# cure-lab/MagicDrive

Measured on NVIDIA H100. Metric: 6-view 224x400 denoising-steps/sec, higher is better.
Workload: dtype bf16

## Files before the change

### magicdrive_b200/csrc/attention_wgmma.cuh

```cuda
#pragma once
#include "ptx.cuh"
#include "wgmma.cuh"

namespace mdb {

constexpr int ATT_BM = 128;

constexpr int ATT_MAX_SRC = 3;
struct AttnKvMaps {
  CUtensorMap k[ATT_MAX_SRC], v[ATT_MAX_SRC];
};

struct AttnParams {
  __nv_bfloat16* out;
  int ldo;
  int lq, lk;
  const int* kv_index;
  int n_sets;
  const int* kv_len;
  int n_src;
  float scale_log2;
  int q_step;
};

template <int D, int BN_ = 0>
struct AttnCfg {
  static constexpr int KD = (D + 63) / 64;
  static constexpr int D16 = (D + 15) / 16 * 16;
  static constexpr int BN = BN_ ? BN_ : ((D16 <= 64) ? 128 : 64);
  static constexpr int TILE_Q = ATT_BM * 128;
  static constexpr int TILE_KV = BN * 128;
  static constexpr int SMEM_Q = KD * TILE_Q;
  static constexpr int STAGES_FIT = (232448 - 1024 - 256 - SMEM_Q) / (2 * KD * TILE_KV);
  static constexpr int STAGES = STAGES_FIT > 4 ? 4 : STAGES_FIT;
  static constexpr int SMEM_KV = STAGES * 2 * KD * TILE_KV;
  static constexpr int kSmemBytes = SMEM_Q + SMEM_KV + 1024 + 256;
  static constexpr int kConsumerWarps = 8;
  static constexpr int kThreads = 32 * kConsumerWarps + 32;
  static constexpr int SACC = BN / 2;
  static constexpr int OACC = D16 / 2;
  static_assert(STAGES >= 1 && kSmemBytes <= 232448, "shared memory");
};

template <int D, int BN_, bool CAUSAL = false>
__global__ void __launch_bounds__(AttnCfg<D, BN_>::kThreads, 1)
attention_wgmma_kernel(const __grid_constant__ CUtensorMap tmQ, const __grid_constant__ AttnKvMaps kvm, const AttnParams p) {
  using Cfg = AttnCfg<D, BN_>;
  constexpr int KD = Cfg::KD, D16 = Cfg::D16, BN = Cfg::BN, STAGES = Cfg::STAGES;
  constexpr int TILE_Q = Cfg::TILE_Q, TILE_KV = Cfg::TILE_KV;
  extern __shared__ uint8_t smem_raw[];
  uint8_t* smem = reinterpret_cast<uint8_t*>((reinterpret_cast<uintptr_t>(smem_raw) + 1023) & ~uintptr_t(1023));
  uint8_t* smQ = smem;
  uint8_t* smK = smQ + Cfg::SMEM_Q;
  uint8_t* smV = smK + STAGES * KD * TILE_KV;
  uint64_t* bars = reinterpret_cast<uint64_t*>(smV + STAGES * KD * TILE_KV);
  uint64_t* q_full = bars;
  uint64_t* q_empty = bars + 1;
  uint64_t* kv_full = bars + 2;
  uint64_t* kv_empty = bars + 2 + STAGES;

  const int warp = threadIdx.x >> 5, lane = threadIdx.x & 31;
  const int b = blockIdx.z, head = blockIdx.y;
  const int nq = (p.lq + ATT_BM - 1) / ATT_BM;
  const int q_step = p.q_step > 0 ? p.q_step : nq;
  const int n_own = (nq - static_cast<int>(blockIdx.x) + q_step - 1) / q_step;
  auto q0_of = [&](int o) { return (static_cast<int>(blockIdx.x) + o * q_step) * ATT_BM; };

  if (warp == Cfg::kConsumerWarps && lane == 0) {
    prefetch_tmap(&tmQ);
    for (int i = 0; i < p.n_src; ++i) {
      prefetch_tmap(&kvm.k[i]);
      prefetch_tmap(&kvm.v[i]);
    }
    mbar_init(q_full, 1);
    mbar_init(q_empty, Cfg::kConsumerWarps);
    for (int i = 0; i < STAGES; ++i) {
      mbar_init(&kv_full[i], 1);
      mbar_init(&kv_empty[i], Cfg::kConsumerWarps);
    }
    fence_barrier_init();
  }
  __syncthreads();
  asm volatile("griddepcontrol.wait;" ::: "memory");
  asm volatile("griddepcontrol.launch_dependents;" ::: "memory");
  const int lkb = p.kv_len ? min(max(p.kv_len[b], 0), p.lk) : p.lk;
  const int ntiles = (lkb + BN - 1) / BN;
  const bool kv_resident = ntiles == 1 && p.n_sets == 1 && n_own > 1;
  auto kv_entry = [&](int set) { return p.kv_index ? p.kv_index[b * p.n_sets + set] : b; };
  auto tiles_of = [&](int kve, int q0) {
    return kve < 0 ? 0 : CAUSAL ? min(ntiles, (min(q0 + ATT_BM, p.lq) - 1) / BN + 1) : ntiles;
  };

  if (warp == Cfg::kConsumerWarps) {
    if (lane == 0) {
      int stage = 0;
      uint32_t phase = 0;
      for (int o = 0; o < n_own; ++o) {
        if (o > 0) mbar_wait(q_empty, static_cast<uint32_t>(o - 1) & 1u);
        mbar_arrive_expect_tx(q_full, KD * TILE_Q);
#pragma unroll
        for (int c = 0; c < KD; ++c) tma_load_4d(&tmQ, q_full, smQ + c * TILE_Q, c * 64, head, q0_of(o), b);
        if (kv_resident && o > 0) continue;
        for (int set = 0; set < p.n_sets; ++set) {
          const int kve = kv_entry(set);
          const int nt = tiles_of(kve, q0_of(o));
          if (nt == 0) continue;
          const int kvb = kve & 0xffffff;
          const CUtensorMap* km = &kvm.k[kve >> 24];
          const CUtensorMap* vm = &kvm.v[kve >> 24];
          for (int j = 0; j < nt; ++j) {
            mbar_wait(&kv_empty[stage], phase ^ 1);
            mbar_arrive_expect_tx(&kv_full[stage], 2 * KD * TILE_KV);
#pragma unroll
            for (int c = 0; c < KD; ++c) {
              tma_load_4d(km, &kv_full[stage], smK + (stage * KD + c) * TILE_KV, c * 64, head, j * BN, kvb);
              tma_load_4d(vm, &kv_full[stage], smV + (stage * KD + c) * TILE_KV, c * 64, head, j * BN, kvb);
            }
            if (++stage == STAGES) {
              stage = 0;
              phase ^= 1;
            }
          }
        }
      }
    }
    return;
  }

  const int wg = warp >> 2;
  const int q = lane & 3;
  const int rloc = 64 * wg + 16 * (warp & 3) + (lane >> 2);
  const float sc = p.scale_log2;
  int stage = 0;
  uint32_t phase = 0;
  for (int o = 0; o < n_own; ++o) {
    const int q0 = q0_of(o);
    mbar_wait(q_full, static_cast<uint32_t>(o) & 1u);
    bool wrote = false;
    for (int set = 0; set < p.n_sets; ++set) {
      const int nt = tiles_of(kv_entry(set), q0);
      if (nt == 0) continue;
      float oacc[Cfg::OACC];
#pragma unroll
      for (int i = 0; i < Cfg::OACC; ++i) oacc[i] = 0.f;
      float m[2] = {-INFINITY, -INFINITY}, l[2] = {0.f, 0.f};
      for (int j = 0; j < nt; ++j) {
        const int st = kv_resident ? 0 : stage;
        mbar_wait(&kv_full[st], kv_resident ? 0u : phase);
        float s[Cfg::SACC];
        wgmma_fence();
#pragma unroll
        for (int k = 0; k < D16 / 16; ++k) {
          const int c = k / 4, kk = k % 4;
          const uint64_t adesc = make_sw128_kmajor_desc(smem_u32(smQ + c * TILE_Q + wg * (64 * 128))) + 2 * kk;
          const uint64_t bdesc = make_sw128_kmajor_desc(smem_u32(smK + (st * KD + c) * TILE_KV)) + 2 * kk;
          WgmmaSS<BN>::run(s, adesc, bdesc, k > 0 ? 1u : 0u);
        }
        wgmma_commit();
        wgmma_wait<0>();
        const int kbase = j * BN;
        if (kbase + BN > lkb) {
#pragma unroll
          for (int g = 0; g < BN / 8; ++g)
#pragma unroll
            for (int e = 0; e < 2; ++e)
              if (kbase + 8 * g + 2 * q + e >= lkb) s[4 * g + e] = s[4 * g + 2 + e] = -INFINITY;
        }
        if constexpr (CAUSAL) {
          if (kbase + BN - 1 > q0 + rloc) {
#pragma unroll
            for (int g = 0; g < BN / 8; ++g)
#pragma unroll
              for (int h = 0; h < 2; ++h)
#pragma unroll
                for (int e = 0; e < 2; ++e)
                  if (kbase + 8 * g + 2 * q + e > q0 + rloc + 8 * h) s[4 * g + 2 * h + e] = -INFINITY;
          }
        }
        float corr[2];
#pragma unroll
        for (int h = 0; h < 2; ++h) {
          float mx = -INFINITY;
#pragma unroll
          for (int g = 0; g < BN / 8; ++g) mx = fmaxf(mx, fmaxf(s[4 * g + 2 * h], s[4 * g + 2 * h + 1]));
          mx = fmaxf(mx, __shfl_xor_sync(0xffffffffu, mx, 1));
          mx = fmaxf(mx, __shfl_xor_sync(0xffffffffu, mx, 2));
          const float m_new = fmaxf(m[h], mx * sc);
          corr[h] = exp2f(m[h] - m_new);
          m[h] = m_new;
        }
        uint32_t pa[BN / 16][4];
        float rs[2] = {0.f, 0.f};
#pragma unroll
        for (int kk = 0; kk < BN / 16; ++kk) {
#pragma unroll
          for (int r = 0; r < 4; ++r) {
            const int h = r & 1;
            const int i0 = 8 * kk + 4 * (r >> 1) + 2 * h;
            const float p0 = exp2f(fmaf(s[i0], sc, -m[h]));
            const float p1 = exp2f(fmaf(s[i0 + 1], sc, -m[h]));
            rs[h] += p0 + p1;
            pa[kk][r] = pack_bf16(p0, p1);
          }
        }
#pragma unroll
        for (int h = 0; h < 2; ++h) l[h] = l[h] * corr[h] + rs[h];
#pragma unroll
        for (int g = 0; g < D16 / 8; ++g) {
          oacc[4 * g] *= corr[0], oacc[4 * g + 1] *= corr[0];
          oacc[4 * g + 2] *= corr[1], oacc[4 * g + 3] *= corr[1];
        }
        wgmma_fence();
#pragma unroll
        for (int kk = 0; kk < BN / 16; ++kk) {
          const uint64_t bdesc = make_sw128_mnmajor_desc(smem_u32(smV + st * KD * TILE_KV), TILE_KV) + (2048u >> 4) * kk;
          WgmmaRSBmn<D16>::run(oacc, pa[kk], bdesc, 1u);
        }
        wgmma_commit();
        wgmma_wait<0>();
        if (!kv_resident) {
          if (lane == 0) mbar_arrive(&kv_empty[stage]);
          if (++stage == STAGES) {
            stage = 0;
            phase ^= 1;
          }
        }
      }
#pragma unroll
      for (int h = 0; h < 2; ++h) {
        l[h] += __shfl_xor_sync(0xffffffffu, l[h], 1);
        l[h] += __shfl_xor_sync(0xffffffffu, l[h], 2);
      }
      const float inv[2] = {1.0f / l[0], 1.0f / l[1]};
#pragma unroll
      for (int h = 0; h < 2; ++h) {
        const int qrow = q0 + rloc + 8 * h;
        if (qrow >= p.lq) continue;
        __nv_bfloat16* orow = p.out + (static_cast<long long>(b) * p.lq + qrow) * p.ldo + head * D;
#pragma unroll
        for (int g = 0; g < D16 / 8; ++g) {
          const int col = 8 * g + 2 * q;
          if (col >= D) continue;
          float f0 = oacc[4 * g + 2 * h] * inv[h], f1 = oacc[4 * g + 2 * h + 1] * inv[h];
          if (wrote) {
            const float2 pf = __bfloat1622float2(*reinterpret_cast<const __nv_bfloat162*>(orow + col));
            f0 = __bfloat162float(__float2bfloat16_rn(f0)) + pf.x;
            f1 = __bfloat162float(__float2bfloat16_rn(f1)) + pf.y;
          }
          *reinterpret_cast<uint32_t*>(orow + col) = pack_bf16(f0, f1);
        }
      }
      wrote = true;
    }
    if (!wrote) {
#pragma unroll
      for (int h = 0; h < 2; ++h) {
        const int qrow = q0 + rloc + 8 * h;
        if (qrow >= p.lq) continue;
        __nv_bfloat16* orow = p.out + (static_cast<long long>(b) * p.lq + qrow) * p.ldo + head * D;
#pragma unroll
        for (int g = 0; g < D16 / 8; ++g)
          if (8 * g + 2 * q < D) *reinterpret_cast<uint32_t*>(orow + 8 * g + 2 * q) = 0u;
      }
    }
    __syncwarp();
    if (lane == 0) mbar_arrive(q_empty);
  }
}

}
```

### magicdrive_b200/csrc/ptx.cuh

```cuda
#pragma once
#include <cuda.h>
#include <cuda_bf16.h>
#include <cuda_runtime.h>
#include <stdint.h>

namespace mdb {

__device__ __forceinline__ uint32_t smem_u32(const void* p) {
  return static_cast<uint32_t>(__cvta_generic_to_shared(p));
}

__device__ __forceinline__ bool elect_one() {
  uint32_t pred = 0;
  asm volatile(
      "{\n\t"
      ".reg .pred P;\n\t"
      "elect.sync _|P, 0xffffffff;\n\t"
      "selp.b32 %0, 1, 0, P;\n\t"
      "}\n"
      : "=r"(pred));
  return pred != 0;
}

__device__ __forceinline__ void mbar_init(uint64_t* bar, uint32_t count) {
  asm volatile("mbarrier.init.shared::cta.b64 [%0], %1;" ::"r"(smem_u32(bar)), "r"(count));
}
__device__ __forceinline__ void fence_barrier_init() {
  asm volatile("fence.mbarrier_init.release.cluster;" ::: "memory");
}
__device__ __forceinline__ void fence_proxy_async() {
  asm volatile("fence.proxy.async.shared::cta;" ::: "memory");
}
__device__ __forceinline__ bool mbar_test(uint64_t* bar, uint32_t parity) {
  uint32_t ok;
  asm volatile(
      "{\n\t"
      ".reg .pred P1;\n\t"
      "mbarrier.test_wait.parity.shared::cta.b64 P1, [%1], %2;\n\t"
      "selp.u32 %0, 1, 0, P1;\n\t"
      "}\n"
      : "=r"(ok)
      : "r"(smem_u32(bar)), "r"(parity)
      : "memory");
  return ok != 0;
}
__device__ __forceinline__ void mbar_arrive_expect_tx(uint64_t* bar, uint32_t bytes) {
  asm volatile("mbarrier.arrive.expect_tx.shared::cta.b64 _, [%0], %1;" ::"r"(smem_u32(bar)), "r"(bytes)
               : "memory");
}
__device__ __forceinline__ void mbar_arrive(uint64_t* bar) {
  asm volatile("mbarrier.arrive.shared::cta.b64 _, [%0];" ::"r"(smem_u32(bar)) : "memory");
}
#ifndef MDB_MBAR_WAIT_MODE
#define MDB_MBAR_WAIT_MODE 0
#endif
__device__ __forceinline__ void mbar_wait(uint64_t* bar, uint32_t parity) {
#if MDB_MBAR_WAIT_MODE == 0
  asm volatile(
      "{\n\t"
      ".reg .pred P1;\n\t"
      "WAIT_LOOP:\n\t"
      "mbarrier.try_wait.parity.shared::cta.b64 P1, [%0], %1, 0x989680;\n\t"
      "@P1 bra DONE;\n\t"
      "bra WAIT_LOOP;\n\t"
      "DONE:\n\t"
      "}\n" ::"r"(smem_u32(bar)),
      "r"(parity)
      : "memory");
#elif MDB_MBAR_WAIT_MODE == 1
  asm volatile(
      "{\n\t"
      ".reg .pred P1;\n\t"
      "WAIT_LOOP:\n\t"
      "mbarrier.try_wait.parity.shared::cta.b64 P1, [%0], %1;\n\t"
      "@P1 bra DONE;\n\t"
      "bra WAIT_LOOP;\n\t"
      "DONE:\n\t"
      "}\n" ::"r"(smem_u32(bar)),
      "r"(parity)
      : "memory");
#else
  asm volatile(
      "{\n\t"
      ".reg .pred P1;\n\t"
      "WAIT_LOOP:\n\t"
      "mbarrier.test_wait.parity.shared::cta.b64 P1, [%0], %1;\n\t"
      "@P1 bra DONE;\n\t"
      "bra WAIT_LOOP;\n\t"
      "DONE:\n\t"
      "}\n" ::"r"(smem_u32(bar)),
      "r"(parity)
      : "memory");
#endif
}

__device__ __forceinline__ void prefetch_tmap(const CUtensorMap* m) {
  asm volatile("prefetch.tensormap [%0];" ::"l"(reinterpret_cast<uint64_t>(m)) : "memory");
}
__device__ __forceinline__ void tma_load_2d(const CUtensorMap* m, uint64_t* bar, void* dst, int c0, int c1) {
  asm volatile(
      "cp.async.bulk.tensor.2d.shared::cluster.global.mbarrier::complete_tx::bytes"
      " [%0], [%1, {%3, %4}], [%2];" ::"r"(smem_u32(dst)),
      "l"(reinterpret_cast<uint64_t>(m)), "r"(smem_u32(bar)), "r"(c0), "r"(c1)
      : "memory");
}
__device__ __forceinline__ void tma_load_4d(const CUtensorMap* m, uint64_t* bar, void* dst, int c0, int c1, int c2,
                                            int c3) {
  asm volatile(
      "cp.async.bulk.tensor.4d.shared::cluster.global.mbarrier::complete_tx::bytes"
      " [%0], [%1, {%3, %4, %5, %6}], [%2];" ::"r"(smem_u32(dst)),
      "l"(reinterpret_cast<uint64_t>(m)), "r"(smem_u32(bar)), "r"(c0), "r"(c1), "r"(c2), "r"(c3)
      : "memory");
}
__device__ __forceinline__ void tma_load_im2col_4d(const CUtensorMap* m, uint64_t* bar, void* dst, int c, int w, int h,
                                                   int n, uint16_t off_w, uint16_t off_h) {
  asm volatile(
      "cp.async.bulk.tensor.4d.shared::cluster.global.im2col.mbarrier::complete_tx::bytes"
      " [%0], [%1, {%3, %4, %5, %6}], [%2], {%7, %8};" ::"r"(smem_u32(dst)),
      "l"(reinterpret_cast<uint64_t>(m)), "r"(smem_u32(bar)), "r"(c), "r"(w), "r"(h), "r"(n), "h"(off_w), "h"(off_h)
      : "memory");
}

__device__ __forceinline__ uint64_t make_sw128_kmajor_desc(uint32_t smem_addr_bytes) {
  uint64_t d = 0;
  d |= static_cast<uint64_t>((smem_addr_bytes >> 4) & 0x3FFF);
  d |= static_cast<uint64_t>(1) << 16;
  d |= static_cast<uint64_t>((1024u >> 4) & 0x3FFF) << 32;
  d |= static_cast<uint64_t>(1) << 62;
  return d;
}
__device__ __forceinline__ uint64_t make_sw128_mnmajor_desc(uint32_t smem_addr_bytes, uint32_t lbo_bytes) {
  uint64_t d = 0;
  d |= static_cast<uint64_t>((smem_addr_bytes >> 4) & 0x3FFF);
  d |= static_cast<uint64_t>((lbo_bytes >> 4) & 0x3FFF) << 16;
  d |= static_cast<uint64_t>((1024u >> 4) & 0x3FFF) << 32;
  d |= static_cast<uint64_t>(1) << 62;
  return d;
}

__device__ __forceinline__ uint32_t pack_bf16(float a, float b) {
  __nv_bfloat162 h = __floats2bfloat162_rn(a, b);
  return *reinterpret_cast<uint32_t*>(&h);
}

}
```

### magicdrive_b200/csrc/wgmma.cuh

```cuda
#pragma once
#include <stdint.h>

namespace mdb {

__device__ __forceinline__ void wgmma_fence() { asm volatile("wgmma.fence.sync.aligned;" ::: "memory"); }
__device__ __forceinline__ void wgmma_commit() { asm volatile("wgmma.commit_group.sync.aligned;" ::: "memory"); }
template <int N>
__device__ __forceinline__ void wgmma_wait() {
  asm volatile("wgmma.wait_group.sync.aligned %0;" ::"n"(N) : "memory");
}

__device__ __forceinline__ void wgmma_ss_n64(float (&d)[32], uint64_t adesc, uint64_t bdesc, uint32_t accumulate) {
  asm volatile(
      "{\n\t.reg .pred p;\n\t"
      "setp.ne.b32 p, %34, 0;\n\t"
      "wgmma.mma_async.sync.aligned.m64n64k16.f32.bf16.bf16 "
      "{%0, %1, %2, %3, %4, %5, %6, %7, %8, %9, %10, %11, %12, %13, %14, %15, %16, %17, %18, %19, %20, %21, %22, %23, %24, %25, %26, %27, %28, %29, %30, %31}, "
      "%32, %33, p, 1, 1, 0, 0;\n\t}\n"
      : "+f"(d[0]), "+f"(d[1]), "+f"(d[2]), "+f"(d[3]), "+f"(d[4]), "+f"(d[5]), "+f"(d[6]), "+f"(d[7]), "+f"(d[8]), "+f"(d[9]), "+f"(d[10]), "+f"(d[11]), "+f"(d[12]), "+f"(d[13]), "+f"(d[14]), "+f"(d[15]), "+f"(d[16]), "+f"(d[17]), "+f"(d[18]), "+f"(d[19]), "+f"(d[20]), "+f"(d[21]), "+f"(d[22]), "+f"(d[23]), "+f"(d[24]), "+f"(d[25]), "+f"(d[26]), "+f"(d[27]), "+f"(d[28]), "+f"(d[29]), "+f"(d[30]), "+f"(d[31])
      : "l"(adesc), "l"(bdesc), "r"(accumulate));
}

__device__ __forceinline__ void wgmma_ss_n128(float (&d)[64], uint64_t adesc, uint64_t bdesc, uint32_t accumulate) {
  asm volatile(
      "{\n\t.reg .pred p;\n\t"
      "setp.ne.b32 p, %66, 0;\n\t"
      "wgmma.mma_async.sync.aligned.m64n128k16.f32.bf16.bf16 "
      "{%0, %1, %2, %3, %4, %5, %6, %7, %8, %9, %10, %11, %12, %13, %14, %15, %16, %17, %18, %19, %20, %21, %22, %23, %24, %25, %26, %27, %28, %29, %30, %31, %32, %33, %34, %35, %36, %37, %38, %39, %40, %41, %42, %43, %44, %45, %46, %47, %48, %49, %50, %51, %52, %53, %54, %55, %56, %57, %58, %59, %60, %61, %62, %63}, "
      "%64, %65, p, 1, 1, 0, 0;\n\t}\n"
      : "+f"(d[0]), "+f"(d[1]), "+f"(d[2]), "+f"(d[3]), "+f"(d[4]), "+f"(d[5]), "+f"(d[6]), "+f"(d[7]), "+f"(d[8]), "+f"(d[9]), "+f"(d[10]), "+f"(d[11]), "+f"(d[12]), "+f"(d[13]), "+f"(d[14]), "+f"(d[15]), "+f"(d[16]), "+f"(d[17]), "+f"(d[18]), "+f"(d[19]), "+f"(d[20]), "+f"(d[21]), "+f"(d[22]), "+f"(d[23]), "+f"(d[24]), "+f"(d[25]), "+f"(d[26]), "+f"(d[27]), "+f"(d[28]), "+f"(d[29]), "+f"(d[30]), "+f"(d[31]), "+f"(d[32]), "+f"(d[33]), "+f"(d[34]), "+f"(d[35]), "+f"(d[36]), "+f"(d[37]), "+f"(d[38]), "+f"(d[39]), "+f"(d[40]), "+f"(d[41]), "+f"(d[42]), "+f"(d[43]), "+f"(d[44]), "+f"(d[45]), "+f"(d[46]), "+f"(d[47]), "+f"(d[48]), "+f"(d[49]), "+f"(d[50]), "+f"(d[51]), "+f"(d[52]), "+f"(d[53]), "+f"(d[54]), "+f"(d[55]), "+f"(d[56]), "+f"(d[57]), "+f"(d[58]), "+f"(d[59]), "+f"(d[60]), "+f"(d[61]), "+f"(d[62]), "+f"(d[63])
      : "l"(adesc), "l"(bdesc), "r"(accumulate));
}

__device__ __forceinline__ void wgmma_ss_n160(float (&d)[80], uint64_t adesc, uint64_t bdesc, uint32_t accumulate) {
  asm volatile(
      "{\n\t.reg .pred p;\n\t"
      "setp.ne.b32 p, %82, 0;\n\t"
      "wgmma.mma_async.sync.aligned.m64n160k16.f32.bf16.bf16 "
      "{%0, %1, %2, %3, %4, %5, %6, %7, %8, %9, %10, %11, %12, %13, %14, %15, %16, %17, %18, %19, %20, %21, %22, %23, %24, %25, %26, %27, %28, %29, %30, %31, %32, %33, %34, %35, %36, %37, %38, %39, %40, %41, %42, %43, %44, %45, %46, %47, %48, %49, %50, %51, %52, %53, %54, %55, %56, %57, %58, %59, %60, %61, %62, %63, %64, %65, %66, %67, %68, %69, %70, %71, %72, %73, %74, %75, %76, %77, %78, %79}, "
      "%80, %81, p, 1, 1, 0, 0;\n\t}\n"
      : "+f"(d[0]), "+f"(d[1]), "+f"(d[2]), "+f"(d[3]), "+f"(d[4]), "+f"(d[5]), "+f"(d[6]), "+f"(d[7]), "+f"(d[8]), "+f"(d[9]), "+f"(d[10]), "+f"(d[11]), "+f"(d[12]), "+f"(d[13]), "+f"(d[14]), "+f"(d[15]), "+f"(d[16]), "+f"(d[17]), "+f"(d[18]), "+f"(d[19]), "+f"(d[20]), "+f"(d[21]), "+f"(d[22]), "+f"(d[23]), "+f"(d[24]), "+f"(d[25]), "+f"(d[26]), "+f"(d[27]), "+f"(d[28]), "+f"(d[29]), "+f"(d[30]), "+f"(d[31]), "+f"(d[32]), "+f"(d[33]), "+f"(d[34]), "+f"(d[35]), "+f"(d[36]), "+f"(d[37]), "+f"(d[38]), "+f"(d[39]), "+f"(d[40]), "+f"(d[41]), "+f"(d[42]), "+f"(d[43]), "+f"(d[44]), "+f"(d[45]), "+f"(d[46]), "+f"(d[47]), "+f"(d[48]), "+f"(d[49]), "+f"(d[50]), "+f"(d[51]), "+f"(d[52]), "+f"(d[53]), "+f"(d[54]), "+f"(d[55]), "+f"(d[56]), "+f"(d[57]), "+f"(d[58]), "+f"(d[59]), "+f"(d[60]), "+f"(d[61]), "+f"(d[62]), "+f"(d[63]), "+f"(d[64]), "+f"(d[65]), "+f"(d[66]), "+f"(d[67]), "+f"(d[68]), "+f"(d[69]), "+f"(d[70]), "+f"(d[71]), "+f"(d[72]), "+f"(d[73]), "+f"(d[74]), "+f"(d[75]), "+f"(d[76]), "+f"(d[77]), "+f"(d[78]), "+f"(d[79])
      : "l"(adesc), "l"(bdesc), "r"(accumulate));
}

__device__ __forceinline__ void wgmma_ss_n256(float (&d)[128], uint64_t adesc, uint64_t bdesc, uint32_t accumulate) {
  asm volatile(
      "{\n\t.reg .pred p;\n\t"
      "setp.ne.b32 p, %130, 0;\n\t"
      "wgmma.mma_async.sync.aligned.m64n256k16.f32.bf16.bf16 "
      "{%0, %1, %2, %3, %4, %5, %6, %7, %8, %9, %10, %11, %12, %13, %14, %15, %16, %17, %18, %19, %20, %21, %22, %23, %24, %25, %26, %27, %28, %29, %30, %31, %32, %33, %34, %35, %36, %37, %38, %39, %40, %41, %42, %43, %44, %45, %46, %47, %48, %49, %50, %51, %52, %53, %54, %55, %56, %57, %58, %59, %60, %61, %62, %63, %64, %65, %66, %67, %68, %69, %70, %71, %72, %73, %74, %75, %76, %77, %78, %79, %80, %81, %82, %83, %84, %85, %86, %87, %88, %89, %90, %91, %92, %93, %94, %95, %96, %97, %98, %99, %100, %101, %102, %103, %104, %105, %106, %107, %108, %109, %110, %111, %112, %113, %114, %115, %116, %117, %118, %119, %120, %121, %122, %123, %124, %125, %126, %127}, "
      "%128, %129, p, 1, 1, 0, 0;\n\t}\n"
      : "+f"(d[0]), "+f"(d[1]), "+f"(d[2]), "+f"(d[3]), "+f"(d[4]), "+f"(d[5]), "+f"(d[6]), "+f"(d[7]), "+f"(d[8]), "+f"(d[9]), "+f"(d[10]), "+f"(d[11]), "+f"(d[12]), "+f"(d[13]), "+f"(d[14]), "+f"(d[15]), "+f"(d[16]), "+f"(d[17]), "+f"(d[18]), "+f"(d[19]), "+f"(d[20]), "+f"(d[21]), "+f"(d[22]), "+f"(d[23]), "+f"(d[24]), "+f"(d[25]), "+f"(d[26]), "+f"(d[27]), "+f"(d[28]), "+f"(d[29]), "+f"(d[30]), "+f"(d[31]), "+f"(d[32]), "+f"(d[33]), "+f"(d[34]), "+f"(d[35]), "+f"(d[36]), "+f"(d[37]), "+f"(d[38]), "+f"(d[39]), "+f"(d[40]), "+f"(d[41]), "+f"(d[42]), "+f"(d[43]), "+f"(d[44]), "+f"(d[45]), "+f"(d[46]), "+f"(d[47]), "+f"(d[48]), "+f"(d[49]), "+f"(d[50]), "+f"(d[51]), "+f"(d[52]), "+f"(d[53]), "+f"(d[54]), "+f"(d[55]), "+f"(d[56]), "+f"(d[57]), "+f"(d[58]), "+f"(d[59]), "+f"(d[60]), "+f"(d[61]), "+f"(d[62]), "+f"(d[63]), "+f"(d[64]), "+f"(d[65]), "+f"(d[66]), "+f"(d[67]), "+f"(d[68]), "+f"(d[69]), "+f"(d[70]), "+f"(d[71]), "+f"(d[72]), "+f"(d[73]), "+f"(d[74]), "+f"(d[75]), "+f"(d[76]), "+f"(d[77]), "+f"(d[78]), "+f"(d[79]), "+f"(d[80]), "+f"(d[81]), "+f"(d[82]), "+f"(d[83]), "+f"(d[84]), "+f"(d[85]), "+f"(d[86]), "+f"(d[87]), "+f"(d[88]), "+f"(d[89]), "+f"(d[90]), "+f"(d[91]), "+f"(d[92]), "+f"(d[93]), "+f"(d[94]), "+f"(d[95]), "+f"(d[96]), "+f"(d[97]), "+f"(d[98]), "+f"(d[99]), "+f"(d[100]), "+f"(d[101]), "+f"(d[102]), "+f"(d[103]), "+f"(d[104]), "+f"(d[105]), "+f"(d[106]), "+f"(d[107]), "+f"(d[108]), "+f"(d[109]), "+f"(d[110]), "+f"(d[111]), "+f"(d[112]), "+f"(d[113]), "+f"(d[114]), "+f"(d[115]), "+f"(d[116]), "+f"(d[117]), "+f"(d[118]), "+f"(d[119]), "+f"(d[120]), "+f"(d[121]), "+f"(d[122]), "+f"(d[123]), "+f"(d[124]), "+f"(d[125]), "+f"(d[126]), "+f"(d[127])
      : "l"(adesc), "l"(bdesc), "r"(accumulate));
}

__device__ __forceinline__ void wgmma_rs_n32_bmn(float (&d)[16], const uint32_t (&a)[4], uint64_t bdesc, uint32_t accumulate) {
  asm volatile(
      "{\n\t.reg .pred p;\n\t"
      "setp.ne.b32 p, %21, 0;\n\t"
      "wgmma.mma_async.sync.aligned.m64n32k16.f32.bf16.bf16 "
      "{%0, %1, %2, %3, %4, %5, %6, %7, %8, %9, %10, %11, %12, %13, %14, %15}, "
      "{%16, %17, %18, %19}, %20, p, 1, 1, 1;\n\t}\n"
      : "+f"(d[0]), "+f"(d[1]), "+f"(d[2]), "+f"(d[3]), "+f"(d[4]), "+f"(d[5]), "+f"(d[6]), "+f"(d[7]), "+f"(d[8]), "+f"(d[9]), "+f"(d[10]), "+f"(d[11]), "+f"(d[12]), "+f"(d[13]), "+f"(d[14]), "+f"(d[15])
      : "r"(a[0]), "r"(a[1]), "r"(a[2]), "r"(a[3]), "l"(bdesc), "r"(accumulate));
}

__device__ __forceinline__ void wgmma_rs_n48_bmn(float (&d)[24], const uint32_t (&a)[4], uint64_t bdesc, uint32_t accumulate) {
  asm volatile(
      "{\n\t.reg .pred p;\n\t"
      "setp.ne.b32 p, %29, 0;\n\t"
      "wgmma.mma_async.sync.aligned.m64n48k16.f32.bf16.bf16 "
      "{%0, %1, %2, %3, %4, %5, %6, %7, %8, %9, %10, %11, %12, %13, %14, %15, %16, %17, %18, %19, %20, %21, %22, %23}, "
      "{%24, %25, %26, %27}, %28, p, 1, 1, 1;\n\t}\n"
      : "+f"(d[0]), "+f"(d[1]), "+f"(d[2]), "+f"(d[3]), "+f"(d[4]), "+f"(d[5]), "+f"(d[6]), "+f"(d[7]), "+f"(d[8]), "+f"(d[9]), "+f"(d[10]), "+f"(d[11]), "+f"(d[12]), "+f"(d[13]), "+f"(d[14]), "+f"(d[15]), "+f"(d[16]), "+f"(d[17]), "+f"(d[18]), "+f"(d[19]), "+f"(d[20]), "+f"(d[21]), "+f"(d[22]), "+f"(d[23])
      : "r"(a[0]), "r"(a[1]), "r"(a[2]), "r"(a[3]), "l"(bdesc), "r"(accumulate));
}

__device__ __forceinline__ void wgmma_rs_n64_bmn(float (&d)[32], const uint32_t (&a)[4], uint64_t bdesc, uint32_t accumulate) {
  asm volatile(
      "{\n\t.reg .pred p;\n\t"
      "setp.ne.b32 p, %37, 0;\n\t"
      "wgmma.mma_async.sync.aligned.m64n64k16.f32.bf16.bf16 "
      "{%0, %1, %2, %3, %4, %5, %6, %7, %8, %9, %10, %11, %12, %13, %14, %15, %16, %17, %18, %19, %20, %21, %22, %23, %24, %25, %26, %27, %28, %29, %30, %31}, "
      "{%32, %33, %34, %35}, %36, p, 1, 1, 1;\n\t}\n"
      : "+f"(d[0]), "+f"(d[1]), "+f"(d[2]), "+f"(d[3]), "+f"(d[4]), "+f"(d[5]), "+f"(d[6]), "+f"(d[7]), "+f"(d[8]), "+f"(d[9]), "+f"(d[10]), "+f"(d[11]), "+f"(d[12]), "+f"(d[13]), "+f"(d[14]), "+f"(d[15]), "+f"(d[16]), "+f"(d[17]), "+f"(d[18]), "+f"(d[19]), "+f"(d[20]), "+f"(d[21]), "+f"(d[22]), "+f"(d[23]), "+f"(d[24]), "+f"(d[25]), "+f"(d[26]), "+f"(d[27]), "+f"(d[28]), "+f"(d[29]), "+f"(d[30]), "+f"(d[31])
      : "r"(a[0]), "r"(a[1]), "r"(a[2]), "r"(a[3]), "l"(bdesc), "r"(accumulate));
}

__device__ __forceinline__ void wgmma_rs_n80_bmn(float (&d)[40], const uint32_t (&a)[4], uint64_t bdesc, uint32_t accumulate) {
  asm volatile(
      "{\n\t.reg .pred p;\n\t"
      "setp.ne.b32 p, %45, 0;\n\t"
      "wgmma.mma_async.sync.aligned.m64n80k16.f32.bf16.bf16 "
      "{%0, %1, %2, %3, %4, %5, %6, %7, %8, %9, %10, %11, %12, %13, %14, %15, %16, %17, %18, %19, %20, %21, %22, %23, %24, %25, %26, %27, %28, %29, %30, %31, %32, %33, %34, %35, %36, %37, %38, %39}, "
      "{%40, %41, %42, %43}, %44, p, 1, 1, 1;\n\t}\n"
      : "+f"(d[0]), "+f"(d[1]), "+f"(d[2]), "+f"(d[3]), "+f"(d[4]), "+f"(d[5]), "+f"(d[6]), "+f"(d[7]), "+f"(d[8]), "+f"(d[9]), "+f"(d[10]), "+f"(d[11]), "+f"(d[12]), "+f"(d[13]), "+f"(d[14]), "+f"(d[15]), "+f"(d[16]), "+f"(d[17]), "+f"(d[18]), "+f"(d[19]), "+f"(d[20]), "+f"(d[21]), "+f"(d[22]), "+f"(d[23]), "+f"(d[24]), "+f"(d[25]), "+f"(d[26]), "+f"(d[27]), "+f"(d[28]), "+f"(d[29]), "+f"(d[30]), "+f"(d[31]), "+f"(d[32]), "+f"(d[33]), "+f"(d[34]), "+f"(d[35]), "+f"(d[36]), "+f"(d[37]), "+f"(d[38]), "+f"(d[39])
      : "r"(a[0]), "r"(a[1]), "r"(a[2]), "r"(a[3]), "l"(bdesc), "r"(accumulate));
}

__device__ __forceinline__ void wgmma_rs_n160_bmn(float (&d)[80], const uint32_t (&a)[4], uint64_t bdesc, uint32_t accumulate) {
  asm volatile(
      "{\n\t.reg .pred p;\n\t"
      "setp.ne.b32 p, %85, 0;\n\t"
      "wgmma.mma_async.sync.aligned.m64n160k16.f32.bf16.bf16 "
      "{%0, %1, %2, %3, %4, %5, %6, %7, %8, %9, %10, %11, %12, %13, %14, %15, %16, %17, %18, %19, %20, %21, %22, %23, %24, %25, %26, %27, %28, %29, %30, %31, %32, %33, %34, %35, %36, %37, %38, %39, %40, %41, %42, %43, %44, %45, %46, %47, %48, %49, %50, %51, %52, %53, %54, %55, %56, %57, %58, %59, %60, %61, %62, %63, %64, %65, %66, %67, %68, %69, %70, %71, %72, %73, %74, %75, %76, %77, %78, %79}, "
      "{%80, %81, %82, %83}, %84, p, 1, 1, 1;\n\t}\n"
      : "+f"(d[0]), "+f"(d[1]), "+f"(d[2]), "+f"(d[3]), "+f"(d[4]), "+f"(d[5]), "+f"(d[6]), "+f"(d[7]), "+f"(d[8]), "+f"(d[9]), "+f"(d[10]), "+f"(d[11]), "+f"(d[12]), "+f"(d[13]), "+f"(d[14]), "+f"(d[15]), "+f"(d[16]), "+f"(d[17]), "+f"(d[18]), "+f"(d[19]), "+f"(d[20]), "+f"(d[21]), "+f"(d[22]), "+f"(d[23]), "+f"(d[24]), "+f"(d[25]), "+f"(d[26]), "+f"(d[27]), "+f"(d[28]), "+f"(d[29]), "+f"(d[30]), "+f"(d[31]), "+f"(d[32]), "+f"(d[33]), "+f"(d[34]), "+f"(d[35]), "+f"(d[36]), "+f"(d[37]), "+f"(d[38]), "+f"(d[39]), "+f"(d[40]), "+f"(d[41]), "+f"(d[42]), "+f"(d[43]), "+f"(d[44]), "+f"(d[45]), "+f"(d[46]), "+f"(d[47]), "+f"(d[48]), "+f"(d[49]), "+f"(d[50]), "+f"(d[51]), "+f"(d[52]), "+f"(d[53]), "+f"(d[54]), "+f"(d[55]), "+f"(d[56]), "+f"(d[57]), "+f"(d[58]), "+f"(d[59]), "+f"(d[60]), "+f"(d[61]), "+f"(d[62]), "+f"(d[63]), "+f"(d[64]), "+f"(d[65]), "+f"(d[66]), "+f"(d[67]), "+f"(d[68]), "+f"(d[69]), "+f"(d[70]), "+f"(d[71]), "+f"(d[72]), "+f"(d[73]), "+f"(d[74]), "+f"(d[75]), "+f"(d[76]), "+f"(d[77]), "+f"(d[78]), "+f"(d[79])
      : "r"(a[0]), "r"(a[1]), "r"(a[2]), "r"(a[3]), "l"(bdesc), "r"(accumulate));
}

template <int N> struct WgmmaSS;
template <> struct WgmmaSS<64> { static __device__ __forceinline__ void run(float (&d)[32], uint64_t a, uint64_t b, uint32_t acc) { wgmma_ss_n64(d, a, b, acc); } };
template <> struct WgmmaSS<128> { static __device__ __forceinline__ void run(float (&d)[64], uint64_t a, uint64_t b, uint32_t acc) { wgmma_ss_n128(d, a, b, acc); } };
template <> struct WgmmaSS<160> { static __device__ __forceinline__ void run(float (&d)[80], uint64_t a, uint64_t b, uint32_t acc) { wgmma_ss_n160(d, a, b, acc); } };
template <> struct WgmmaSS<256> { static __device__ __forceinline__ void run(float (&d)[128], uint64_t a, uint64_t b, uint32_t acc) { wgmma_ss_n256(d, a, b, acc); } };
template <int N> struct WgmmaRSBmn;
template <> struct WgmmaRSBmn<32> { static __device__ __forceinline__ void run(float (&d)[16], const uint32_t (&a)[4], uint64_t b, uint32_t acc) { wgmma_rs_n32_bmn(d, a, b, acc); } };
template <> struct WgmmaRSBmn<48> { static __device__ __forceinline__ void run(float (&d)[24], const uint32_t (&a)[4], uint64_t b, uint32_t acc) { wgmma_rs_n48_bmn(d, a, b, acc); } };
template <> struct WgmmaRSBmn<64> { static __device__ __forceinline__ void run(float (&d)[32], const uint32_t (&a)[4], uint64_t b, uint32_t acc) { wgmma_rs_n64_bmn(d, a, b, acc); } };
template <> struct WgmmaRSBmn<80> { static __device__ __forceinline__ void run(float (&d)[40], const uint32_t (&a)[4], uint64_t b, uint32_t acc) { wgmma_rs_n80_bmn(d, a, b, acc); } };
template <> struct WgmmaRSBmn<160> { static __device__ __forceinline__ void run(float (&d)[80], const uint32_t (&a)[4], uint64_t b, uint32_t acc) { wgmma_rs_n160_bmn(d, a, b, acc); } };

}
```

Before: 56.57.

## Overlap next QK wgmma with PV in attention, add register reallocation and double-buffered Q

```diff
diff --git a/magicdrive_b200/csrc/attention_wgmma.cuh b/magicdrive_b200/csrc/attention_wgmma.cuh
--- a/magicdrive_b200/csrc/attention_wgmma.cuh
+++ b/magicdrive_b200/csrc/attention_wgmma.cuh
@@ -1,4 +1,6 @@
 #pragma once
+#include <type_traits>
+
 #include "ptx.cuh"
 #include "wgmma.cuh"
 
@@ -36,7 +38,11 @@
   static constexpr int SMEM_KV = STAGES * 2 * KD * TILE_KV;
   static constexpr int kSmemBytes = SMEM_Q + SMEM_KV + 1024 + 256;
   static constexpr int kConsumerWarps = 8;
-  static constexpr int kThreads = 32 * kConsumerWarps + 32;
+  static constexpr int kThreads = 32 * kConsumerWarps + 128;
+  static constexpr int kProducerRegs = 24, kConsumerRegs = 240;
+  static_assert(128 * kProducerRegs + 32 * kConsumerWarps * kConsumerRegs <= 65536, "register file");
+  static constexpr bool kAhead = STAGES >= 2;
+  static constexpr bool kQ2 = (STAGES - 1) * BN >= ATT_BM;
   static constexpr int SACC = BN / 2;
   static constexpr int OACC = D16 / 2;
   static_assert(STAGES >= 1 && kSmemBytes <= 232448, "shared memory");
@@ -55,9 +61,9 @@
   uint8_t* smV = smK + STAGES * KD * TILE_KV;
   uint64_t* bars = reinterpret_cast<uint64_t*>(smV + STAGES * KD * TILE_KV);
   uint64_t* q_full = bars;
-  uint64_t* q_empty = bars + 1;
-  uint64_t* kv_full = bars + 2;
-  uint64_t* kv_empty = bars + 2 + STAGES;
+  uint64_t* q_empty = bars + 2;
+  uint64_t* kv_full = bars + 4;
+  uint64_t* kv_empty = bars + 4 + STAGES;
 
   const int warp = threadIdx.x >> 5, lane = threadIdx.x & 31;
   const int b = blockIdx.z, head = blockIdx.y;
@@ -72,8 +78,10 @@
       prefetch_tmap(&kvm.k[i]);
       prefetch_tmap(&kvm.v[i]);
     }
-    mbar_init(q_full, 1);
-    mbar_init(q_empty, Cfg::kConsumerWarps);
+    for (int i = 0; i < 2; ++i) {
+      mbar_init(&q_full[i], 1);
+      mbar_init(&q_empty[i], Cfg::kConsumerWarps);
+    }
     for (int i = 0; i < STAGES; ++i) {
       mbar_init(&kv_full[i], 1);
       mbar_init(&kv_empty[i], Cfg::kConsumerWarps);
@@ -86,20 +94,24 @@
   const int lkb = p.kv_len ? min(max(p.kv_len[b], 0), p.lk) : p.lk;
   const int ntiles = (lkb + BN - 1) / BN;
   const bool kv_resident = ntiles == 1 && p.n_sets == 1 && n_own > 1;
+  const int nqb = kv_resident && Cfg::kQ2 ? 2 : 1;
+  auto q_buf = [&](int o) { return o % nqb ? smK + KD * TILE_KV : smQ; };
   auto kv_entry = [&](int set) { return p.kv_index ? p.kv_index[b * p.n_sets + set] : b; };
   auto tiles_of = [&](int kve, int q0) {
     return kve < 0 ? 0 : CAUSAL ? min(ntiles, (min(q0 + ATT_BM, p.lq) - 1) / BN + 1) : ntiles;
   };
 
-  if (warp == Cfg::kConsumerWarps) {
-    if (lane == 0) {
+  if (warp >= Cfg::kConsumerWarps) {
+    setmaxnreg_dec<Cfg::kProducerRegs>();
+    if (warp == Cfg::kConsumerWarps && lane == 0) {
       int stage = 0;
       uint32_t phase = 0;
       for (int o = 0; o < n_own; ++o) {
-        if (o > 0) mbar_wait(q_empty, static_cast<uint32_t>(o - 1) & 1u);
-        mbar_arrive_expect_tx(q_full, KD * TILE_Q);
-#pragma unroll
-        for (int c = 0; c < KD; ++c) tma_load_4d(&tmQ, q_full, smQ + c * TILE_Q, c * 64, head, q0_of(o), b);
+        const int qb = o % nqb, use = o / nqb;
+        if (use > 0) mbar_wait(&q_empty[qb], static_cast<uint32_t>(use - 1) & 1u);
+        mbar_arrive_expect_tx(&q_full[qb], KD * TILE_Q);
+#pragma unroll
+        for (int c = 0; c < KD; ++c) tma_load_4d(&tmQ, &q_full[qb], q_buf(o) + c * TILE_Q, c * 64, head, q0_of(o), b);
         if (kv_resident && o > 0) continue;
         for (int set = 0; set < p.n_sets; ++set) {
           const int kve = kv_entry(set);
@@ -127,15 +139,49 @@
     return;
   }
 
+  setmaxnreg_inc<Cfg::kConsumerRegs>();
   const int wg = warp >> 2;
   const int q = lane & 3;
   const int rloc = 64 * wg + 16 * (warp & 3) + (lane >> 2);
   const float sc = p.scale_log2;
   int stage = 0;
   uint32_t phase = 0;
+  int rel = 0;
+  auto acquire = [&]() {
+    if (kv_resident) {
+      mbar_wait(&kv_full[0], 0u);
+      return 0;
+    }
+    const int st = stage;
+    mbar_wait(&kv_full[st], phase);
+    if (++stage == STAGES) {
+      stage = 0;
+      phase ^= 1;
+    }
+    return st;
+  };
+  auto release = [&]() {
+    if (kv_resident) return;
+    if (lane == 0) mbar_arrive(&kv_empty[rel]);
+    if (++rel == STAGES) rel = 0;
+  };
+  uint8_t* sq = smQ;
+  auto issue_qk = [&](float (&s)[Cfg::SACC], int st) {
+    wgmma_fence();
+#pragma unroll
+    for (int k = 0; k < D16 / 16; ++k) {
+      const int c = k / 4, kk = k % 4;
+      const uint64_t adesc = make_sw128_kmajor_desc(smem_u32(sq + c * TILE_Q + wg * (64 * 128))) + 2 * kk;
+      const uint64_t bdesc = make_sw128_kmajor_desc(smem_u32(smK + (st * KD + c) * TILE_KV)) + 2 * kk;
+      WgmmaSS<BN>::run(s, adesc, bdesc, k > 0 ? 1u : 0u);
+    }
+    wgmma_commit();
+  };
   for (int o = 0; o < n_own; ++o) {
     const int q0 = q0_of(o);
-    mbar_wait(q_full, static_cast<uint32_t>(o) & 1u);
+    const int qb = o % nqb;
+    mbar_wait(&q_full[qb], static_cast<uint32_t>(o / nqb) & 1u);
+    sq = q_buf(o);
     bool wrote = false;
     for (int set = 0; set < p.n_sets; ++set) {
       const int nt = tiles_of(kv_entry(set), q0);
@@ -144,20 +190,14 @@
 #pragma unroll
       for (int i = 0; i < Cfg::OACC; ++i) oacc[i] = 0.f;
       float m[2] = {-INFINITY, -INFINITY}, l[2] = {0.f, 0.f};
-      for (int j = 0; j < nt; ++j) {
-        const int st = kv_resident ? 0 : stage;
-        mbar_wait(&kv_full[st], kv_resident ? 0u : phase);
-        float s[Cfg::SACC];
-        wgmma_fence();
-#pragma unroll
-        for (int k = 0; k < D16 / 16; ++k) {
-          const int c = k / 4, kk = k % 4;
-          const uint64_t adesc = make_sw128_kmajor_desc(smem_u32(smQ + c * TILE_Q + wg * (64 * 128))) + 2 * kk;
-          const uint64_t bdesc = make_sw128_kmajor_desc(smem_u32(smK + (st * KD + c) * TILE_KV)) + 2 * kk;
-          WgmmaSS<BN>::run(s, adesc, bdesc, k > 0 ? 1u : 0u);
-        }
-        wgmma_commit();
-        wgmma_wait<0>();
+      float s[Cfg::SACC];
+      uint32_t pa[BN / 16][4];
+      int st = acquire();
+      issue_qk(s, st);
+      wgmma_wait<0>();
+      wgmma_fence_operand(s);
+      auto key_tile = [&](auto More, int j) {
+        constexpr bool more = decltype(More)::value;
         const int kbase = j * BN;
         if (kbase + BN > lkb) {
 #pragma unroll
@@ -189,7 +229,6 @@
           corr[h] = exp2f(m[h] - m_new);
           m[h] = m_new;
         }
-        uint32_t pa[BN / 16][4];
         float rs[2] = {0.f, 0.f};
 #pragma unroll
         for (int kk = 0; kk < BN / 16; ++kk) {
@@ -200,32 +239,56 @@
             const float p0 = exp2f(fmaf(s[i0], sc, -m[h]));
             const float p1 = exp2f(fmaf(s[i0 + 1], sc, -m[h]));
             rs[h] += p0 + p1;
-            pa[kk][r] = pack_bf16(p0, p1);
+            s[i0] = p0, s[i0 + 1] = p1;
           }
         }
 #pragma unroll
         for (int h = 0; h < 2; ++h) l[h] = l[h] * corr[h] + rs[h];
+        wgmma_wait<0>();
+        wgmma_fence_operand(oacc);
+        if (Cfg::kAhead && j > 0) release();
 #pragma unroll
         for (int g = 0; g < D16 / 8; ++g) {
           oacc[4 * g] *= corr[0], oacc[4 * g + 1] *= corr[0];
           oacc[4 * g + 2] *= corr[1], oacc[4 * g + 3] *= corr[1];
         }
+#pragma unroll
+        for (int kk = 0; kk < BN / 16; ++kk) {
+          wgmma_fence_operand(pa[kk]);
+#pragma unroll
+          for (int r = 0; r < 4; ++r) {
+            const int i0 = 8 * kk + 4 * (r >> 1) + 2 * (r & 1);
+            pa[kk][r] = pack_bf16(s[i0], s[i0 + 1]);
+          }
+        }
+        const int st_j = st;
+        if constexpr (more && Cfg::kAhead) {
+          st = acquire();
+          issue_qk(s, st);
+        }
         wgmma_fence();
 #pragma unroll
         for (int kk = 0; kk < BN / 16; ++kk) {
-          const uint64_t bdesc = make_sw128_mnmajor_desc(smem_u32(smV + st * KD * TILE_KV), TILE_KV) + (2048u >> 4) * kk;
+          const uint64_t bdesc = make_sw128_mnmajor_desc(smem_u32(smV + st_j * KD * TILE_KV), TILE_KV) + (2048u >> 4) * kk;
           WgmmaRSBmn<D16>::run(oacc, pa[kk], bdesc, 1u);
         }
         wgmma_commit();
-        wgmma_wait<0>();
-        if (!kv_resident) {
-          if (lane == 0) mbar_arrive(&kv_empty[stage]);
-          if (++stage == STAGES) {
-            stage = 0;
-            phase ^= 1;
-          }
-        }
-      }
+        if constexpr (more) {
+          if constexpr (!Cfg::kAhead) {
+            wgmma_wait<0>();
+            release();
+            st = acquire();
+            issue_qk(s, st);
+          }
+          wgmma_wait<Cfg::kAhead ? 1 : 0>();
+          wgmma_fence_operand(s);
+        }
+      };
+      for (int j = 0; j + 1 < nt; ++j) key_tile(std::true_type(), j);
+      key_tile(std::false_type(), nt - 1);
+      wgmma_wait<0>();
+      wgmma_fence_operand(oacc);
+      release();
 #pragma unroll
       for (int h = 0; h < 2; ++h) {
         l[h] += __shfl_xor_sync(0xffffffffu, l[h], 1);
@@ -264,7 +327,7 @@
       }
     }
     __syncwarp();
-    if (lane == 0) mbar_arrive(q_empty);
+    if (lane == 0) mbar_arrive(&q_empty[qb]);
   }
 }
 
diff --git a/magicdrive_b200/csrc/ptx.cuh b/magicdrive_b200/csrc/ptx.cuh
--- a/magicdrive_b200/csrc/ptx.cuh
+++ b/magicdrive_b200/csrc/ptx.cuh
@@ -138,6 +138,15 @@
   return d;
 }
 
+template <uint32_t N>
+__device__ __forceinline__ void setmaxnreg_dec() {
+  asm volatile("setmaxnreg.dec.sync.aligned.u32 %0;" ::"n"(N));
+}
+template <uint32_t N>
+__device__ __forceinline__ void setmaxnreg_inc() {
+  asm volatile("setmaxnreg.inc.sync.aligned.u32 %0;" ::"n"(N));
+}
+
 __device__ __forceinline__ uint32_t pack_bf16(float a, float b) {
   __nv_bfloat162 h = __floats2bfloat162_rn(a, b);
   return *reinterpret_cast<uint32_t*>(&h);
diff --git a/magicdrive_b200/csrc/wgmma.cuh b/magicdrive_b200/csrc/wgmma.cuh
--- a/magicdrive_b200/csrc/wgmma.cuh
+++ b/magicdrive_b200/csrc/wgmma.cuh
@@ -8,6 +8,16 @@
 template <int N>
 __device__ __forceinline__ void wgmma_wait() {
   asm volatile("wgmma.wait_group.sync.aligned %0;" ::"n"(N) : "memory");
+}
+template <int N>
+__device__ __forceinline__ void wgmma_fence_operand(float (&r)[N]) {
+#pragma unroll
+  for (int i = 0; i < N; ++i) asm volatile("" : "+f"(r[i])::"memory");
+}
+template <int N>
+__device__ __forceinline__ void wgmma_fence_operand(uint32_t (&r)[N]) {
+#pragma unroll
+  for (int i = 0; i < N; ++i) asm volatile("" : "+r"(r[i])::"memory");
 }
 
 __device__ __forceinline__ void wgmma_ss_n64(float (&d)[32], uint64_t adesc, uint64_t bdesc, uint32_t accumulate) {
```

After: 57.03, median of 6. Within noise of the previous version (+0.8%).
